# flybirdxx/ComfyUI-SDMatte

Measured on AMD Instinct MI355X. Metric: alpha mattes/sec at 1024x1024, higher is better.
Workload: dtype f16x3

## Files before the change

comfyui-sdmatte_amd/csrc/k_gemm.h:

```cpp
#pragma once
#include "sdm_common.h"

#ifndef P3_X8_TRUNC_GAIN
#define P3_X8_TRUNC_GAIN 1.097f
#endif

SDM_DEV_INLINE int p3_xl_pos(int c) { const int j = c >> 3; return ((j & 1) << 4) | ((j >> 1) << 3) | (c & 7); }
SDM_HD_INLINE size_t p3_rows_pad(size_t rows) { return (rows + 31) & ~(size_t)31; }
SDM_DEV_INLINE size_t p3_hi_off(size_t row, int C, int c) {
  return ((((row >> 4) * (size_t)(C >> 5)) + (size_t)(c >> 5)) << 10) + (size_t)((((c & 31) >> 3) << 8) + ((int)(row & 15) << 4));
}
SDM_DEV_INLINE size_t p3_xl_off(size_t row, int C, int c) {
  const int pos = p3_xl_pos(c & 31);
  return ((((row >> 5) * (size_t)(C >> 5)) + (size_t)(c >> 5)) << 10) + (size_t)(((pos >> 4) << 9) + ((int)(row & 31) << 4) + (pos & 15));
}

SDM_DEV_INLINE float p3_gelu(float g) {
  const float z = fabsf(g) * 0.70710678118654752f;
  const float t = sdm_rcp(1.0f + 0.3275911f * z);
  const float poly = t * (0.254829592f + t * (-0.284496736f + t * (1.421413741f + t * (-1.453152027f + t * 1.061405429f))));
  const float er = 1.0f - poly * sdm_exp2(-z * z * SDM_LOG2E);
  return 0.5f * g * (1.0f + copysignf(er, g));
}

// ... 1 lines not shown
  const half_t* a_hi; const unsigned char* a_xl;
  long M; int K;
  int rows_per_img;
  const unsigned char* w; int N;
  const float* bias;
  void* out; int ldo;
  int n_valid;
  size_t out_lo_off;
  int lo_cols;
  const float* res; int ldr;
  float* stats;
  int sa, sb;
  int tiles_m, tiles_n, xcd_chunk, tiles_per_img;
  int ablate;
  int up_H, up_W;
};

SDM_DEV_INLINE void p3_pack_block(const float (&v)[16], u32x4 (&hi)[2], u32x4& xl) {
  unsigned int H[4][2], X[4];
#pragma unroll
  for (int g = 0; g < 4; ++g) {
    float y[4], l[4];
    half_t hh[4];
#pragma unroll
    for (int e = 0; e < 4; ++e) {
      y[e] = SDM_MED3(v[4 * g + e], -57344.0f, 57344.0f);
      hh[e] = (half_t)y[e];
      l[e] = (y[e] - (float)hh[e]) * 2048.0f;
    }
    f16x2 p0, p1;
// ... 372 lines not shown
          const u32x4 hv = {H[2 * q][0], H[2 * q][1], H[2 * q + 1][0], H[2 * q + 1][1]};
          const u32x4 pv = {P[2 * q][0], P[2 * q][1], P[2 * q + 1][0], P[2 * q + 1][1]};
          sdm_buffer_store16(hv, rs_hi, ok ? (ro + (unsigned int)ch) * 2u : SDM_BUF_INVALID, 0);
          SDM_PIN_STORE_DATA(hv);
          sdm_buffer_store16(pv, rs_pr, (ok && ch < p.lo_cols) ? (ro + (unsigned int)ch) * 2u : SDM_BUF_INVALID, 0);
          SDM_PIN_STORE_DATA(pv);
        }
      }
    }
  }
  }
  v_cur = next_tile(v_cur + (int)gridDim.x, mt_c, nt_c);
  }
}

SDM_DEV_INLINE float up_phase_weight(const half_t* __restrict__ k_hi, const half_t* __restrict__ k_lo, int Cout_pad, int phase, int tap, int c, int co) {
  const int py = phase >> 1, px = phase & 1, a = tap >> 1, b = tap & 1;
  float s = 0.0f;
  for (int ky = 0; ky < 3; ++ky) {
    if (((py + ky + 1) >> 1) - 1 != py - 1 + a) continue;
    for (int kx = 0; kx < 3; ++kx) {
      if (((px + kx + 1) >> 1) - 1 != px - 1 + b) continue;
      const size_t si = (((size_t)(c / 16) * 9 + ky * 3 + kx) * Cout_pad + co) * 16 + (c % 16);
      s += (float)k_hi[si] + (float)k_lo[si];
    }
  }
  return s;
}
__global__ void up_phase_absmax_kernel(const half_t* __restrict__ k_hi, const half_t* __restrict__ k_lo, int Cin_pad, int Cout_pad, unsigned int* __restrict__ out) {
  const size_t n = (size_t)16 * Cin_pad * Cout_pad;
// ... 201 lines not shown
```

comfyui-sdmatte_amd/csrc/sdm_engine.cpp:

```cpp
#include "sdm_common.h"
#include "k_conv.h"
#include "k_gemm.h"
#include "k_norm.h"
#include "k_attn.h"
#include "k_misc.h"
#include "k_trimap.h"
#include "k_cclabel.h"
#include "k_foreground.h"
#include "k_guided.h"
#include "k_roi.h"
#include "k_canvas.h"
#include "k_boxes.h"
#include "k_distance.h"
#include "../../include/sdmatte.h"

#include <algorithm>
#include <cmath>
#include <cstdio>
#include <cstdlib>
#include <cstring>
#include <atomic>
#include <map>
#include <mutex>
#include <shared_mutex>
// ... 48 lines not shown
}
#endif
static inline size_t rupz(size_t a, size_t b) { return ((a + b - 1) / b) * b; }

struct OptEntry { const char* name; int value; int def; const char* what; };
static OptEntry g_opts[] = {
  {"conv_f8", 1, 1, "residual terms of the wide split-precision 3x3 convs on fp8 MFMAs (read when a model is built)"},
  {"gemm_f8", 1, 1, "the same for Linear / 1x1 layers with K >= gemm_f8_min_k (read when a model is built)"},
  {"gemm_f8_min_k", 1024, 1024, "smallest K of a GEMM that takes the 8-wave fp8-residual kernel"},
  {"gemm_p3", 1, 1, "transformer-block Linear layers on the plane-fed GEMM (k_gemm.h): pre-split operand planes from LayerNorm / GroupNorm / attention / GEGLU, LDS-DMA only (the W3 weight copies are built when a model is built)"},
  {"gemm_p3_tile", 0, 0, "row tile of the plane-fed GEMM: 0 by shape, 256 / 128 / 64 forced"},
  {"gemm_p3_attn", 1, 1, "d=64 attention cores write the operand planes of to_out themselves (0: fp32 result + one conversion pass)"},
  {"gemm_p3_persist", 1, 1, "plane-fed GEMM: persistent blocks that prefetch the next tile's first chunk underneath the epilogue (0: one block per tile, n > 1: a grid of n blocks - tests)"},
  {"gemm_p3_ablate", 0, 0, "bench only: 1 no MFMAs, 2 no DMAs behind the prologue, 4 no epilogue (sdm_bench_gemm_p3)"},
  {"conv_up_phase", 1, 1, "up-sampling 3x3 convs (Upsample2D) as four 2x2-tap phase convs on the plane-fed GEMM (k_gemm.h, UP): 0 off (the 3x3 kernels on the up-sampled image), 1 the launches with at least two 256-row tiles per CU (up_phase_wins: measured), 2 every eligible launch (tests).  0 / non-0 is read when a model is built: the phase matrices are a derived weight layout"},
  {"conv_epi", 4, 4, "F8 kernels' epilogue: 4 register-direct stores + residual as accumulator init, 3 residual init only, 0 LDS-staged"},
  {"conv_xtile", 1, 1, "F8 3x3: cross-tile prefetch by the producer waves"},
  {"conv_f8_tpb", 0, 0, "F8: tiles per block (0 = by queue depth)"},
  {"conv_dma", 1, 1, "3x3 stride-1 256x128 tile: weights by LDS-DMA"},
  {"conv_dma_all", 0, 0, "keep a stage-ordered weight copy for every wide 3x3 layer, not only the split-precision ones (read when a model is built)"},
  {"conv_pc", -1, -1, "producer / consumer form of the split-precision DMA kernel: -1 by channel count, 0 off, 1 on"},
  {"conv_pc_min_cin", 256, 256, "conv_pc = -1: smallest Cin that takes the producer / consumer form"},
  {"conv_db", 0, 0, "512x128 double-buffered tile where the queue is deep"},
  {"trimap_skip", 1, 1, "VAE encoder, trimap images: output tiles inside a constant region of the trimap are not multiplied (k_misc.h cmask_*; exact). 0 = every tile"},
  {"conv_band_rows", 0, 0, "tile rows per XCD band of the convs that leave constant tiles out (0 = by image height)"},
  {"trimap_skip_min_rows", 512, 512, "smallest output height at which constant tiles are left out (measured at 1024^2: the 1024- and 512-row levels gain 3.7 + 1.6 ms, the 256-row level loses 0.7: too few of its 32 x 128-pixel tiles lie inside one region)"},
  {"conv_splitk", -1, -1, "split-K of the register-staged conv / GEMM kernels: -1 by shape (few tiles, long K), 0 off, n >= 2 forced where the shape allows"},
  {"force_cfg0", 0, 0, "always the 256x128 tile for 3x3 stride 1 (tests: fused GroupNorm at tiny sizes)"},
  {"no_gn_fuse", 0, 0, "never fuse the GroupNorm apply into the consuming conv"},
  {"split_lds_pad", 0, 0, "extra dynamic LDS of the register-staged split kernels (forces one block per CU)"},
// ... 237 lines not shown

template <int MT, int EPI, int UP = 0>
static void launch_gemm_p3_t(GemmP3Params p, void* stream) {
  constexpr int BM = 64 * MT, NS = 2, SMEM = NS * (BM * 96 + 128 * 128);
  const long rows = p.rows_per_img ? (long)p.rows_per_img : p.M;
  p.tiles_per_img = (int)((rows + BM - 1) / BM);
  p.tiles_m = p.tiles_per_img * (p.rows_per_img ? (int)(p.M / p.rows_per_img) : 1);
  p.tiles_n = sdm_cdiv(p.N, 128) * (UP ? 4 : 1);
  unsigned grid;
  if (p.tiles_m >= 8) { p.xcd_chunk = (p.tiles_m + 7) / 8; grid = (unsigned)(8L * p.xcd_chunk * p.tiles_n); }
  else { p.xcd_chunk = 0; grid = (unsigned)(p.tiles_m * p.tiles_n); }
  if (const int pp = opt("gemm_p3_persist")) {
    const unsigned slots = pp > 1 ? (unsigned)pp : ((unsigned)(device_cus() * ((SMEM <= 80 * 1024) ? 2 : 1)) & ~7u);
    if (slots >= 1 && grid > slots) grid = slots;
  }
  auto k = gemm_p3_kernel<MT, 2, EPI, NS, UP>;
  SDM_SET_SMEM(k, SMEM);
#ifndef SDM_EMU
  if (opt("gemm_p3_ablate") & 256) {
    int nb = -1;
    (void)hipOccupancyMaxActiveBlocksPerMultiprocessor(&nb, k, 256, (size_t)SMEM);
    fprintf(stderr, "[gemm_p3] tile %d stages %d epi %d: %d bytes of LDS, %d blocks per CU, grid %u\n", BM, NS, EPI, SMEM, nb, grid);
  }
#endif
  SDM_LAUNCH(k, dim3(grid, 1, 1), dim3(256), (size_t)SMEM, stream, p);
}
template <int EPI>
static void launch_gemm_p3_e(const GemmP3Params& p, int bm, void* stream) {
  if (bm == 256) launch_gemm_p3_t<4, EPI>(p, stream);
  else if (bm == 128) launch_gemm_p3_t<2, EPI>(p, stream);
// ... 7 lines not shown
  const int cus = device_cus();
  for (int bm : {256, 128}) if (imgs * ((rows + bm - 1) / bm) * tn >= cus) return bm;
  return 64;
}
static void launch_gemm_p3(const GemmP3Params& p, int epi, void* stream) {
  const int bm = gemm_p3_pick_bm(p.M, p.N, p.rows_per_img);
  switch (epi) {
    case 0: launch_gemm_p3_e<0>(p, bm, stream); break;
    case 1: launch_gemm_p3_e<1>(p, bm, stream); break;
    case 2: launch_gemm_p3_e<2>(p, bm, stream); break;
    case 3: launch_gemm_p3_e<3>(p, bm, stream); break;
    default: launch_gemm_p3_e<4>(p, bm, stream); break;
  }
}

static void launch_gemm_p3_up(const GemmP3Params& p, int epi, int bm, void* stream) {
  if (epi == 4) {
    if (bm == 256) launch_gemm_p3_t<4, 4, 1>(p, stream); else if (bm == 128) launch_gemm_p3_t<2, 4, 1>(p, stream); else launch_gemm_p3_t<1, 4, 1>(p, stream);
  } else {
    if (bm == 256) launch_gemm_p3_t<4, 0, 1>(p, stream); else if (bm == 128) launch_gemm_p3_t<2, 0, 1>(p, stream); else launch_gemm_p3_t<1, 0, 1>(p, stream);
  }
}

static int launch_conv(int ntaps, int stride, int cfg, const ConvParams& p, void* stream) {
  if (ntaps == 9 && stride == 1) {
    switch (cfg) {
      case 0:
        if (p.w_dma) { launch_conv_dma(p, stream); return 0; }
        launch_conv_t<9, 1, 8, 32, 128, 16, 2, 2, 0, 1>(p, stream); return 0;
      case 1: launch_conv_t<9, 1, 4, 32, 64, 32, 4, 1>(p, stream); return 0;
      case 2: launch_conv_t<9, 1, 8, 8, 64, 16, 2, 1>(p, stream); return 0;
// ... 92 lines not shown
  return L;
}

static bool layer_takes_dma3x3(const ConvL& L) { return L.ntaps == 9 && L.Cout_pad >= 128 && !L.geglu; }
static bool layer_takes_gemm_f8(const ConvL& L) {
  return L.ntaps == 1 && L.split && L.Cout_pad >= 128 && L.Cin_pad % 32 == 0 && conv_f8_enabled() && gemm_f8_enabled();
}
static bool layer_takes_w3(const ConvL& L) { return L.ntaps == 1 && L.split && L.Cin_pad % 32 == 0 && L.Cin_pad >= 32; }
static bool layer_takes_up_phase(const ConvL& L) {
  return L.ntaps == 9 && L.split && !L.geglu && L.Cin_pad % 32 == 0 && L.Cin_pad >= 32 && conv_f8_enabled() && opt("conv_up_phase") != 0;
}
static bool up_phase_wins(int N, int H, int W, int Cout_pad) {
  if (opt("conv_up_phase") >= 2) return true;
  const long tiles = (long)N * sdm_cdiv((H + 2) * (W + 2), 256) * 4 * sdm_cdiv(Cout_pad, 128);
  return tiles >= 2L * device_cus();
}
static void layer_choose_layouts(ConvL& L, bool want_dma3x3, bool want_gemm_f8, bool want_w3, bool want_up_phase = false) {
  if (want_up_phase && layer_takes_up_phase(L)) L.wup_bytes = (size_t)16 * L.Cin_pad * L.Cout_pad * 4;
  if (want_dma3x3 && layer_takes_dma3x3(L)) {
    L.wdma_bytes = L.w_bytes() * (L.split ? 2 : 1);
    L.f8 = (L.split && L.Cin_pad % 32 == 0 && conv_f8_enabled()) ? 1 : 0;
  }
  if (want_gemm_f8 && layer_takes_gemm_f8(L)) { L.wdma_bytes = L.w_bytes() * 2; L.f8 = 1; }
  if (want_w3 && layer_takes_w3(L)) L.w3_bytes = L.w_bytes() * 2;
}
struct NormL {
  int C = 0;
  size_t g_off = 0, b_off = 0;
  float* g = nullptr;
  float* b = nullptr;
// ... 529 lines not shown
  return p3_rows_pad(rows) * (size_t)L.Cin_pad * 2 < SDM_BUF_INVALID && tile_out < SDM_BUF_INVALID && rows < ((size_t)1 << 31);
}
static int op_conv_up_phase(sdm_ctx* e, const ConvL& L, const ConvArgs& a) {
  const T& in = *a.in0;
  T* out = a.out;
  T xp = talloc(e, in.N, in.H + 2, in.W + 2, in.C, kFmtP3);
  GemmP3Params p;
  memset(&p, 0, sizeof(p));
  p.M = xp.rows(); p.K = L.Cin_pad; p.rows_per_img = (in.H + 2) * (in.W + 2);
  p.up_H = in.H; p.up_W = in.W;
  p.a_hi = (const half_t*)xp.p; p.a_xl = (const unsigned char*)xp.p + p3_rows_pad((size_t)p.M) * p.K * 2;
  p.w = L.wup; p.N = L.Cout_pad; p.bias = L.b;
  p.out = out->p; p.ldo = out->C; p.n_valid = a.cout_valid >= 0 ? a.cout_valid : std::min(L.Cout_pad, out->C);
  p.sa = 127 - 11; p.sb = 127 - L.up_exp;
  const int bm = gemm_p3_pick_bm(p.M, p.N, p.rows_per_img, 4);
  const int epi = out->want_stats ? 4 : 0;
  if (epi == 4) {
    out->srows = sdm_cdiv(p.rows_per_img, bm) * 8;
    T sb = talloc(e, 1, 1, 1, (int)((size_t)in.N * out->srows * out->C * 2), 1);
    out->soff = sb.off; out->sbytes = sb.bytes; out->stats = (float*)sb.p;
    p.stats = out->stats;
  }
  if (e->dry) { tfree(e, xp); return 0; }
  char d[256];
  d[0] = 0;
  if (e->prof_on) snprintf(d, sizeof(d), "%s N=%d H=%d W=%d C=%d bordered grid", L.name.c_str(), in.N, in.H, in.W, in.C);
  prof_begin(e, "to_p3", 0, (double)in.rows() * in.C * 4 + (double)xp.rows() * in.C * 3, d);
  const long units = ((xp.rows() + 31) / 32) * (in.C / 32);
  SDM_LAUNCH(to_p3_pad_kernel, dim3((unsigned)std::min<long>((units + 3) / 4, 1 << 20)), dim3(256), 0, e->stream, (const float*)in.p, (unsigned char*)xp.p, xp.rows(), in.C,
             in.H, in.W);
  prof_end(e);
  const double flops = 2.0 * (double)out->rows() * L.O * L.I * 4;
  const double bytes = (double)xp.rows() * p.K * 3 + (double)out->rows() * p.n_valid * 4 + (double)16 * p.K * p.N * 4;
  if (e->prof_on) {
    snprintf(d, sizeof(d), "%s N=%d Hout=%d Wout=%d Cin=%d Cout=%d up=1 phases epi=%d bm=%d", L.name.c_str(), in.N, out->H, out->W, L.Cin_pad, L.O, epi, bm);
    prof_begin(e, "conv_up_phase", flops, bytes, d);
  } else {
    prof_begin(e, "conv", flops, bytes);
  }
  count_kernel("conv_up_phase");
  launch_gemm_p3_up(p, epi, bm, e->stream);
#ifndef SDM_EMU
  { const hipError_t le = hipGetLastError(); if (le != hipSuccess) SDM_FAIL(e, SDM_ERR_HIP, "conv %s: launch failed: %s", L.name.c_str(), hipGetErrorString(le)); }
#endif
  prof_end(e);
  tfree(e, xp);
  return 0;
}

static int op_conv(sdm_ctx* e, const ConvL& L, const ConvArgs& a) {
  if (conv_up_phase_ok(L, a)) return op_conv_up_phase(e, L, a);
  ConvParams p;
  memset(&p, 0, sizeof(p));
  conv_shape_params(p, L, *a.in0, a.in1, *a.out, a.stride);
  p.in0 = a.in0->p;
  if (a.in1) p.in1 = a.in1->p;
// ... 2367 lines not shown
```

comfyui-sdmatte_amd/csrc/sdm_hooks.h:

```cpp
#pragma once

struct DevBuf {
  void* p = nullptr;
  DevBuf() = default;
  DevBuf(DevBuf&& o) noexcept : p(o.p) { o.p = nullptr; }
  ~DevBuf() { if (p) dev_free(p); }
  int alloc(size_t n) { return dev_malloc(&p, n); }
  int alloc0(size_t n, void* stream) { const int rc = alloc(n); return rc ? rc : dev_memset(p, 0, n, stream); }
};

struct RestoreInt { int& s; int v; ~RestoreInt() { s = v; } };

struct TempLayer {
  enum { kDma = 1, kW3 = 2, kUp = 4 };
  sdm_ctx* e;
  ConvL L;
  DevBuf w, w_lo, b, w_dma, w3, wup;
  explicit TempLayer(sdm_ctx* c) : e(c) {}
  ~TempLayer() { dev_sync(e->stream); }
  int init(const char* name, int ntaps, int I, int O, int geglu, int split, int layouts, const float* wsrc, const float* bias) {
    L = make_layer(name, ntaps, I, O, geglu, split);
    layer_choose_layouts(L, layouts & kDma, layouts & kDma, layouts & kW3, layouts & kUp);
    SDM_CHECK_DEV(e, w.alloc0(L.w_bytes(), e->stream));
    SDM_CHECK_DEV(e, b.alloc0(L.b_bytes(), e->stream));
// ... 209 lines not shown
  GemmP3Params p;
  memset(&p, 0, sizeof(p));
  p.M = M; p.K = K; p.a_hi = (const half_t*)xp.p; p.a_xl = (const unsigned char*)xp.p + p3_rows_pad((size_t)M) * K * 2;
  p.w = tl.L.w3; p.N = O; p.bias = tl.L.b; p.out = out.p; p.ldo = Cst; p.n_valid = Cst;
  p.out_lo_off = epi == 2 ? (size_t)M * Cst : p3_rows_pad((size_t)M) * Cst * 2; p.lo_cols = (O / 3) * 2;
  if (resf) { p.res = (const float*)resb.p; p.ldr = Cst; }
  if (epi == 4) { p.stats = (float*)st.p; p.rows_per_img = (int)M; }
  p.sa = 127 - 11; p.sb = 127 - tl.L.f8_exp; p.ablate = opt("gemm_p3_ablate");
  const float ms = time_launches(e, iters, [&]() { launch_gemm_p3(p, epi, e->stream); });
  const hipError_t le = hipGetLastError();
  if (le != hipSuccess) { e->err = hipGetErrorString(le); return -3.f; }
  return ms;
#endif
}

float sdm_bench_conv(sdm_ctx* e, int N, int H, int W, int Cin, int Cout, int ntaps, int stride, int in_f32, int tile_cfg, int ablate, int iters) {
  const int split = (in_f32 >> 1) & 1, gnf = (in_f32 >> 2) & 1, pcf = (in_f32 >> 3) & 1, f8f = (in_f32 >> 4) & 1;
  const int of32 = (in_f32 >> 5) & 1, resf = (in_f32 >> 6) & 1, statf = (in_f32 >> 7) & 1;
  in_f32 = (in_f32 & 1) | split;
  if (e) dev_use(e->device);
  if (!e) return -1.f;
#ifdef SDM_EMU
  return -1.f;
#else
  ConvL L;
  L.name = "bench"; L.ntaps = ntaps; L.I = Cin; L.O = Cout; L.Cin_pad = rup(Cin, 16); L.Cout_pad = rup(Cout, 32);
  DevBuf wp, bp, in, out, wl, gnt, resb, statb, wdm, wsb;
  const int Ho = stride == 2 ? H / 2 : H, Wo = stride == 2 ? W / 2 : W;
  const size_t wbytes = (size_t)L.Cin_pad * ntaps * L.Cout_pad * 2, inb = (size_t)N * H * W * L.Cin_pad * (in_f32 ? 4 : 2),
               outb = (size_t)N * Ho * Wo * L.Cout_pad * (of32 ? 4 : 2);
// ... 372 lines not shown
```

comfyui-sdmatte_amd/engine.py:

```python
import ctypes as C
import os

import numpy as np
import torch

from .config import SDMatteConfig

_HERE = os.path.dirname(os.path.abspath(__file__))
LIB_PATH = os.path.join(_HERE, "csrc", "libsdmatte_hip.so")

SDM_PTR_HOST, SDM_PTR_DEVICE = 0, 1
SDM_F32, SDM_F16, SDM_BF16 = 0, 1, 2
_DT = {torch.float32: SDM_F32, torch.float16: SDM_F16, torch.bfloat16: SDM_BF16}


class SdmConfig(C.Structure):
    _fields_ = [
        ("vae_channels", C.c_int32 * 4), ("vae_layers_per_block", C.c_int32),
        ("unet_channels", C.c_int32 * 4), ("unet_heads", C.c_int32 * 4), ("unet_layers_per_block", C.c_int32),
        ("cross_attention_dim", C.c_int32), ("unet_in_channels", C.c_int32), ("unet_out_channels", C.c_int32),
        ("bbox_embeddings_input_dim", C.c_int32), ("groups", C.c_int32),
        ("vae_eps", C.c_float), ("unet_res_eps", C.c_float), ("unet_tf_gn_eps", C.c_float), ("unet_ln_eps", C.c_float),
        ("vae_scaling_factor", C.c_float), ("attn_mask_value", C.c_float),
        ("stream_f32", C.c_int32), ("point_embeddings_input_dim", C.c_int32), ("precise_mask", C.c_int32), ("reserved", C.c_int32 * 5),
# ... 36 lines not shown
    c.unet_tf_gn_eps, c.unet_ln_eps = cfg.unet_tf_gn_eps, cfg.unet_ln_eps
    c.vae_scaling_factor, c.attn_mask_value = cfg.vae_scaling_factor, cfg.attn_mask_value
    c.stream_f32 = 1 if stream_f32 else 0
    c.point_embeddings_input_dim = cfg.point_embeddings_input_dim
    c.precise_mask = precise_mask_of(precision)
    return c


EXPORTS = [
    "sdm_default_config", "sdm_create", "sdm_destroy", "sdm_last_error", "sdm_load_tensor", "sdm_finalize_weights",
    "sdm_weight_stats", "sdm_missing_key", "sdm_weight_blob_bytes", "sdm_export_weight_blob", "sdm_import_weight_blob",
    "sdm_host_blob_bytes", "sdm_export_host_blob", "sdm_import_host_blob", "sdm_forward", "sdm_forward_ex", "sdm_forward_rect", "sdm_apply_matte", "sdm_apply_matte_node",
    "sdm_make_trimap", "sdm_clean_mask", "sdm_apply_matte_mask", "sdm_subject_roi", "sdm_apply_matte_roi", "sdm_subject_boxes", "sdm_apply_matte_boxes", "sdm_estimate_foreground", "sdm_refine_alpha_guided", "sdm_compose_canvas",
    "sdm_distance_field", "sdm_offset_mask", "sdm_outline",
    "sdm_synchronize", "sdm_release_memory", "sdm_resident_bytes", "sdm_weight_bytes", "sdm_last_forward_ms", "sdm_profile_enable", "sdm_profile_count", "sdm_profile_get", "sdm_profile_dump",
    "sdm_op_conv", "sdm_op_conv_ex", "sdm_op_conv_up_stats", "sdm_op_gemm_p3", "sdm_debug_run_layer", "sdm_debug_set_input_cmask", "sdm_debug_temb_row", "sdm_conv_num_cfgs", "sdm_bench_conv", "sdm_bench_attn", "sdm_bench_gemm_p3", "sdm_op_groupnorm", "sdm_op_layernorm", "sdm_op_attention", "sdm_op_attention_ex", "sdm_op_attention_split", "sdm_op_attention_split_ex", "sdm_debug_attn_plan", "sdm_op_resize_aa",
    "sdm_op_mask_bias", "sdm_op_cross_patch_planes", "sdm_op_cross_patch_planes_ex", "sdm_op_attention_shared", "sdm_debug_cross_attention", "sdm_op_cross_core",
    "sdm_set_option", "sdm_get_option", "sdm_reset_options", "sdm_option_name", "sdm_option_help", "sdm_kernel_counts", "sdm_kernel_counts_reset",
]


class Bindings:

    def __init__(self, cdll):
        self.dll = cdll
        vp, i32, i64, f32 = C.c_void_p, C.c_int, C.c_int64, C.c_float
        sig = {
            "sdm_default_config": (None, [C.POINTER(SdmConfig)]),
            "sdm_create": (i32, [C.POINTER(vp), i32, C.POINTER(SdmConfig)]),
            "sdm_destroy": (None, [vp]),
            "sdm_last_error": (C.c_char_p, [vp]),
# ... 36 lines not shown
            "sdm_profile_get": (i32, [vp, i32, C.POINTER(C.c_char_p), C.POINTER(f32), C.POINTER(i64), C.POINTER(C.c_double),
                                      C.POINTER(C.c_double)]),
            "sdm_op_conv": (i32, [vp, vp, vp, i32, i32, i32, i32, i32, i32, i32, i32, i32, i32, vp, vp, i32, vp, i32, vp, i32, i32,
                                  f32, i32]),
            "sdm_op_conv_ex": (i32, [vp, vp, vp, i32, i32, i32, i32, i32, i32, i32, i32, i32, i32, vp, vp, i32, vp, i32, vp, i32, i32,
                                     f32, i32, i32, vp, vp, f32, i32, i32]),
            "sdm_op_gemm_p3": (i32, [vp, vp, i32, i32, i32, i32, vp, vp, i32, i32, vp, vp, vp, f32, i32, vp, vp, C.POINTER(i32)]),
            "sdm_op_conv_up_stats": (i32, [vp, vp, i32, i32, i32, i32, vp, vp, i32, vp, vp, C.POINTER(i32)]),
            "sdm_debug_run_layer": (i32, [vp, C.c_char_p, vp, i32, i32, i32, vp, i32]),
            "sdm_debug_set_input_cmask": (i32, [vp, vp]),
            "sdm_debug_temb_row": (i32, [vp, i32, i32, vp, vp, i32]),
            "sdm_conv_num_cfgs": (i32, [i32, i32]),
            "sdm_bench_conv": (f32, [vp] + [i32] * 11),
            "sdm_bench_attn": (f32, [vp] + [i32] * 7),
            "sdm_bench_gemm_p3": (f32, [vp, C.c_long, i32, i32, i32, i32]),
            "sdm_op_groupnorm": (i32, [vp, vp, vp, i32, i32, i32, i32, i32, i32, vp, vp, f32, i32, vp]),
            "sdm_op_layernorm": (i32, [vp, vp, i32, C.c_long, i32, vp, vp, f32, vp]),
            "sdm_op_attention": (i32, [vp, vp, i32, vp, i32, vp, i32, vp, i32, i32, i32, i32, i32, vp, i32]),
            "sdm_op_attention_ex": (i32, [vp, vp, i32, vp, i32, vp, i32, i32, i32, i32, i32, i32, i32, vp, i32]),
            "sdm_op_attention_split": (i32, [vp, vp, vp, vp, vp, i32, i32, i32, i32, vp]),
            "sdm_op_attention_split_ex": (i32, [vp, vp, vp, vp, vp, vp, i32, i32, i32, i32, i32, vp, vp]),
            "sdm_debug_attn_plan": (i32, [i32] * 10 + [C.c_char_p, i32, C.POINTER(i32)]),
            "sdm_op_resize_aa": (i32, [vp, vp, i32, i32, i32, vp, i32, i32]),
            "sdm_op_mask_bias": (i32, [vp, vp, i32, i32, i32, vp]),
            "sdm_op_cross_patch_planes": (i32, [vp, vp, i32, i32, i32, vp, vp, vp]),
            "sdm_op_cross_patch_planes_ex": (i32, [vp, vp, i32, i32, i32, vp, vp, vp, i32]),
            "sdm_op_cross_core": (i32, [vp, vp, vp, i32, i32, i32, i32, i32, vp]),
            "sdm_op_attention_shared": (i32, [vp, vp, vp, vp, i32, i32, i32, i32, i32, vp]),
            "sdm_debug_cross_attention": (i32, [vp, C.c_char_p, vp, i32, i32, i32, vp, i32, i32, vp]),
            "sdm_set_option": (i32, [C.c_char_p, i32]),
# ... 760 lines not shown
        return out

    def debug_temb_row(self, index, is_trans, coords, cout):
        out = np.zeros(cout, np.float32)
        co = None if coords is None else np.ascontiguousarray(np.asarray(coords, np.float32).reshape(4))
        self._check(self.lib.sdm_debug_temb_row(self.h, index, int(is_trans), co.ctypes.data_as(C.c_void_p) if co is not None else None,
                                                out.ctypes.data_as(C.c_void_p), cout), "sdm_debug_temb_row")
        return torch.from_numpy(out)

    def bench_conv(self, N, H, W, Cin, Cout, ntaps=9, stride=1, in_f32=0, tile_cfg=-1, ablate=0, iters=10):
        return float(self.lib.sdm_bench_conv(self.h, N, H, W, Cin, Cout, ntaps, stride, in_f32, tile_cfg, ablate, iters))

    def bench_gemm_p3(self, M, K, O, epi=0, res=False, iters=10):
        return float(self.lib.sdm_bench_gemm_p3(self.h, M, K, O, epi | (256 if res else 0), iters))

    def bench_attn(self, B, heads, Lq, Lk, qt=1, ablate=0, iters=10):
        return float(self.lib.sdm_bench_attn(self.h, B, heads, Lq, Lk, qt, ablate, iters))

    def op_groupnorm(self, x0, gamma, beta, eps, silu, groups=32, x1=None):
        N, H, W_, C0 = x0.shape
        C1 = x1.shape[-1] if x1 is not None else 0
        out = torch.empty(N, H, W_, C0 + C1, dtype=torch.float16, device=x0.device)
        self._check(self.lib.sdm_op_groupnorm(self.h, _ptr(x0), _ptr(x1), C0, C1, int(x0.dtype == torch.float32), N, H * W_, groups,
                                              _ptr(gamma), _ptr(beta), float(eps), int(silu), _ptr(out)), "sdm_op_groupnorm")
        return out

    def op_layernorm(self, x, gamma, beta, eps):
        rows, Cc = x.numel() // x.shape[-1], x.shape[-1]
        out = torch.empty(x.shape, dtype=torch.float16, device=x.device)
        self._check(self.lib.sdm_op_layernorm(self.h, _ptr(x), int(x.dtype == torch.float32), rows, Cc, _ptr(gamma), _ptr(beta),
# ... 81 lines not shown
```

include/sdmatte.h:

```cpp
#ifndef SDMATTE_H_
#define SDMATTE_H_

#include <stddef.h>
#include <stdint.h>

#ifdef __cplusplus
extern "C" {
#endif

typedef struct sdm_ctx sdm_ctx;

enum sdm_status {
  SDM_OK = 0,
  SDM_ERR_INVALID = -1,
  SDM_ERR_HIP = -2,
  SDM_ERR_STATE = -3,
  SDM_ERR_NOMEM = -4,
  SDM_ERR_NODEVICE = -5,
  SDM_ERR_ARENA = -6
};

enum sdm_ptr_kind { SDM_PTR_HOST = 0, SDM_PTR_DEVICE = 1 };
enum sdm_dtype { SDM_F32 = 0, SDM_F16 = 1, SDM_BF16 = 2 };

// ... 146 lines not shown
int sdm_profile_enable(sdm_ctx* ctx, int on);
int sdm_profile_count(sdm_ctx* ctx);
const char* sdm_profile_dump(sdm_ctx* ctx);
int sdm_profile_get(sdm_ctx* ctx, int i, const char** name, float* ms, int64_t* launches, double* flops, double* bytes);


int sdm_op_conv(sdm_ctx* ctx, const void* in0, const void* in1, int C0, int C1, int in_f32, int N, int Hin, int Win, int up,
                int stride, int pad_mode, int ntaps, const float* w, const float* bias, int O, void* out, int out_f32,
                const void* res, int res_f32, int geglu, float out_scale, int tile_cfg);
int sdm_conv_num_cfgs(int ntaps, int stride);
int sdm_op_conv_ex(sdm_ctx* ctx, const void* in0, const void* in1, int C0, int C1, int in_f32, int N, int Hin, int Win, int up,
                   int stride, int pad_mode, int ntaps, const float* w, const float* bias, int O, void* out, int out_f32,
                   const void* res, int res_f32, int geglu, float out_scale, int tile_cfg, int split, const float* gn_gamma,
                   const float* gn_beta, float gn_eps, int gn_groups, int gn_silu);
float sdm_bench_gemm_p3(sdm_ctx* ctx, long M, int K, int O, int epi_flags, int iters);
int sdm_op_gemm_p3(sdm_ctx* ctx, const float* x, int N, int H, int W, int K, const float* w, const float* bias, int O, int mode, const float* res,
                   const float* ln_gamma, const float* ln_beta, float ln_eps, int lo_cols, void* out, float* stats, int* srows);
int sdm_op_conv_up_stats(sdm_ctx* ctx, const float* x, int N, int H, int W, int C, const float* w, const float* bias, int O, float* out, float* stats,
                         int* srows);
int sdm_debug_set_input_cmask(sdm_ctx* ctx, const unsigned char* mask);
int sdm_debug_run_layer(sdm_ctx* ctx, const char* layer_name, const float* x_nhwc, int N, int H, int W, float* out_nhwc, int Cout);
int sdm_debug_temb_row(sdm_ctx* ctx, int temb_index, int is_trans, const float* coords4, float* out_host, int cout);
float sdm_bench_attn(sdm_ctx* ctx, int B, int heads, int Lq, int Lk, int qt, int ablate, int iters);
float sdm_bench_conv(sdm_ctx* ctx, int N, int H, int W, int Cin, int Cout, int ntaps, int stride, int in_f32, int tile_cfg, int ablate, int iters);
int sdm_op_groupnorm(sdm_ctx* ctx, const void* in0, const void* in1, int C0, int C1, int in_f32, int N, int HW, int groups,
                     const float* gamma, const float* beta, float eps, int silu, void* out_f16);
int sdm_op_layernorm(sdm_ctx* ctx, const void* x, int in_f32, long rows, int C, const float* gamma, const float* beta,
                     float eps, void* out_f16);
int sdm_op_attention(sdm_ctx* ctx, const void* q, int ldq, const void* k, int ldk, const void* v, int ldv, const float* bias,
                     int B, int heads, int Lq, int Lk, int D, void* out, int ldo);
// ... 20 lines not shown
```

Measured before the change: 21.98.

## Add halo-tile kernel for up-sampling phase convs sharing LDS activations across taps

Adds gemm_p3_up_halo_kernel. It loads one (TH+1)x33 activation halo tile into LDS per channel chunk and reuses it for all four 2x2 taps of a phase conv, instead of reading a separate row tile per tap. This is meant to cut global and LDS-DMA traffic for the activation operand of the Upsample2D convs. It uses a ring of weight slots, tuned vmcnt waits and a statistics layout per spatial tile. The cost is a larger LDS footprint, possibly lower occupancy, and partial tiles at image edges. It is enabled by default for launches with at least two tiles per CU, and also adds a benchmark entry point and a grid-cap test option.

```diff
diff --git a/comfyui-sdmatte_amd/csrc/k_gemm.h b/comfyui-sdmatte_amd/csrc/k_gemm.h
--- a/comfyui-sdmatte_amd/csrc/k_gemm.h
+++ b/comfyui-sdmatte_amd/csrc/k_gemm.h
@@ -39,6 +39,7 @@
   int tiles_m, tiles_n, xcd_chunk, tiles_per_img;
   int ablate;
   int up_H, up_W;
+  int up_tw;
 };
 
 SDM_DEV_INLINE void p3_pack_block(const float (&v)[16], u32x4 (&hi)[2], u32x4& xl) {
@@ -441,6 +442,292 @@
   }
 }
 
+template <int V> struct p3_ic { static constexpr int v = V; };
+template <int N> SDM_DEV_INLINE void p3_wait_vmcnt() {
+#ifndef SDM_EMU
+  asm volatile("s_waitcnt vmcnt(%0)" :: "n"(N) : "memory");
+#endif
+}
+template <int TH, int NW> struct P3HaloCfg {
+  static constexpr int MT = TH / 2, BN = 128;
+  static constexpr int RH = (TH + 1) * 33, ND = (RH + 63) / 64, RPAD = ND * 64;
+  static constexpr int A_HI = 4 * RPAD * 16, A_BUF = 6 * RPAD * 16, W_SLOT = BN * 128, OFF_W = 2 * A_BUF, SMEM = OFF_W + NW * W_SLOT;
+};
+template <int TH, int NW, int EPI>
+__global__ void __launch_bounds__(256, (P3HaloCfg<TH, NW>::SMEM <= 80 * 1024) ? 2 : 1) gemm_p3_up_halo_kernel(GemmP3Params p) {
+  using CF = P3HaloCfg<TH, NW>;
+  constexpr int MT = CF::MT, NT = 2, BN = CF::BN, ND = CF::ND, RPAD = CF::RPAD, RH = CF::RH;
+  constexpr int A_HI = CF::A_HI, A_BUF = CF::A_BUF, W_SLOT = CF::W_SLOT, OFF_W = CF::OFF_W, B_HI = BN * 64;
+  constexpr int AW = (6 * ND + 3) / 4, NXW = AW - ND, NWI = 2 * (BN / 16 / 4);
+  constexpr int AP0 = (AW + 2) / 3, AP1 = (AW + 1) / 3, AP2 = AW / 3;
+  constexpr int AL0 = (NW == 2) ? 0 : NWI, AL1 = (NW == 2) ? AP0 : NWI + AP0, AL2 = (NW == 2) ? AP1 : AP0 + NWI + AP1, AL3 = (NW == 2) ? AP2 : AP1 + NWI + AP2;
+  static_assert(TH % 2 == 0 && (NW == 2 || NW == 3) && AP0 + AP1 + AP2 == AW && NXW >= 1 && NXW * 4 <= 4 * ND && AL2 <= 63 && AL3 <= 63, "halo tile / ring");
+  static_assert(EPI == 0 || EPI == 4, "up-sampling phase convs store fp32 rows");
+  SDM_DYN_SMEM(smem);
+  const int tx = (int)threadIdx.x, lane = tx & 63, wave = SDM_UNIFORM_I(tx >> 6);
+  const int wm = wave >> 1, wn = wave & 1, h = lane >> 5, l31 = lane & 31;
+  const int nchunk = p.K >> 5, nch = nchunk * 4;
+  const unsigned int K = (unsigned int)p.K, N = (unsigned int)p.N;
+  const int up_wp = p.up_W + 2, up_tn = p.tiles_n >> 2;
+  const long rows_pad = (long)p3_rows_pad((size_t)p.M);
+  const int vgrid = (p.xcd_chunk > 0) ? 8 * p.xcd_chunk * p.tiles_n : p.tiles_m * p.tiles_n;
+  auto next_tile = [&](int v, int& mt, int& nt) -> int {
+    for (; v < vgrid; v += (int)gridDim.x) {
+      if (p.xcd_chunk > 0) {
+        const int j = v >> 3, ml = j / p.tiles_n;
+        nt = j - ml * p.tiles_n;
+        mt = (v & 7) * p.xcd_chunk + ml;
+        if (mt < p.tiles_m) return v;
+      } else {
+        mt = v / p.tiles_n;
+        nt = v - mt * p.tiles_n;
+        return v;
+      }
+    }
+    return -1;
+  };
+  auto tile_org = [&](int mt, int& img, int& mti, int& y0, int& x0) {
+    img = mt / p.tiles_per_img; mti = mt - img * p.tiles_per_img;
+    const int tyi = mti / p.up_tw;
+    y0 = tyi * TH; x0 = (mti - tyi * p.up_tw) * 32;
+  };
+  const sdm_rsrc rs_ahi = sdm_make_rsrc(p.a_hi, (unsigned int)rows_pad * K * 2u);
+  const sdm_rsrc rs_axl = sdm_make_rsrc(p.a_xl, (unsigned int)rows_pad * K);
+  const unsigned int vo_w = (unsigned int)lane * 16u;
+
+  unsigned int hi_vo[ND], xl_vo[NXW];
+  int xl_dst[NXW];
+#pragma unroll
+  for (int k = 0; k < NXW; ++k) {
+    int q = k * 4 + wave;
+    if (q >= 2 * ND) q -= 2 * ND;
+    xl_dst[k] = A_HI + (q & 1) * RPAD * 16 + (q >> 1) * 1024;
+  }
+  auto a_setup = [&](int mt, int ph) {
+    int img, mti, y0, x0;
+    tile_org(mt, img, mti, y0, x0);
+    const int yb0 = y0 + (ph >> 1), xb0 = x0 + (ph & 1);
+    auto src_row = [&](int R, bool& ok) -> size_t {
+      const int r = R / 33, s = R - r * 33, yb = yb0 + r, xb = xb0 + s;
+      ok = R < RH && yb <= p.up_H + 1 && xb <= p.up_W + 1;
+      return (size_t)img * p.rows_per_img + (size_t)yb * up_wp + xb;
+    };
+#pragma unroll
+    for (int k = 0; k < ND; ++k) {
+      bool ok;
+      const size_t row = src_row(k * 64 + lane, ok);
+      hi_vo[k] = ok ? (unsigned int)p3_hi_off(row, (int)K, wave * 8) : SDM_BUF_INVALID;
+    }
+#pragma unroll
+    for (int k = 0; k < NXW; ++k) {
+      int q = k * 4 + wave;
+      if (q >= 2 * ND) q -= 2 * ND;
+      bool ok;
+      const size_t row = src_row((q >> 1) * 64 + lane, ok);
+      xl_vo[k] = ok ? (unsigned int)p3_xl_off(row, (int)K, (q & 1) * 8) : SDM_BUF_INVALID;
+    }
+  };
+  int mt_c, nt_c, v_cur = next_tile((int)blockIdx.x, mt_c, nt_c);
+  if (v_cur < 0) return;
+  auto nt_phase = [&](int nt) -> int { return nt / up_tn; };
+  auto nt_col0 = [&](int nt) -> int { return (nt % up_tn) * BN; };
+  int v_a = v_cur, cc_a = 0, par_a = 0;
+  a_setup(mt_c, nt_phase(nt_c));
+  auto issue_a = [&](auto part) {
+    constexpr int T = decltype(part)::v;
+    constexpr int A0 = (T == 0) ? 0 : (T == 1) ? AP0 : AP0 + AP1, AN = (T == 0) ? AP0 : (T == 1) ? AP1 : AP2;
+    if (v_a < 0) return;
+    unsigned char* ab = smem + par_a * A_BUF;
+    const unsigned int add = (unsigned int)cc_a << 10;
+#pragma unroll
+    for (int a = A0; a < A0 + AN; ++a) {
+      if (a < ND) {
+        sdm_glds16_buf(rs_ahi, hi_vo[a] == SDM_BUF_INVALID ? SDM_BUF_INVALID : hi_vo[a] + add, 0u, ab + wave * (RPAD * 16) + a * 1024);
+      } else {
+        sdm_glds16_buf(rs_axl, xl_vo[a - ND] == SDM_BUF_INVALID ? SDM_BUF_INVALID : xl_vo[a - ND] + add, 0u, ab + xl_dst[a - ND]);
+      }
+    }
+    if (T == 2) {
+      par_a ^= 1;
+      if (++cc_a == nchunk) {
+        int mt, nt;
+        cc_a = 0;
+        v_a = next_tile(v_a + (int)gridDim.x, mt, nt);
+        if (v_a >= 0) a_setup(mt, nt_phase(nt));
+      }
+    }
+  };
+  int v_w = v_cur, s_w = 0, slot_w = 0, n0_w = nt_col0(nt_c), ph_w = nt_phase(nt_c);
+  auto issue_w = [&]() {
+    if (v_w < 0) return;
+    unsigned char* st = smem + OFF_W + slot_w * W_SLOT;
+    const sdm_rsrc rs_wc = sdm_make_rsrc(p.w + (size_t)ph_w * ((size_t)nch * N * 128u), (unsigned int)nch * N * 128u);
+    const unsigned int wb = (unsigned int)s_w * N * 128u + (unsigned int)n0_w * 64u;
+#pragma unroll
+    for (int i0 = 0; i0 < BN / 16; i0 += 4) {
+      const int i = i0 + wave;
+      sdm_glds16_buf(rs_wc, vo_w, wb + (unsigned int)i * 1024u, st + i * 1024);
+    }
+#pragma unroll
+    for (int i0 = 0; i0 < BN / 16; i0 += 4) {
+      const int i = i0 + wave;
+      sdm_glds16_buf(rs_wc, vo_w, wb + N * 64u + (unsigned int)i * 1024u, st + B_HI + i * 1024);
+    }
+    slot_w = (slot_w + 1 == NW) ? 0 : slot_w + 1;
+    if (++s_w == nch) {
+      int mt, nt;
+      s_w = 0;
+      v_w = next_tile(v_w + (int)gridDim.x, mt, nt);
+      if (v_w >= 0) { n0_w = nt_col0(nt); ph_w = nt_phase(nt); }
+    }
+  };
+  issue_a(p3_ic<0>()); issue_a(p3_ic<1>()); issue_a(p3_ic<2>());
+#pragma unroll
+  for (int s = 0; s < NW - 1; ++s) issue_w();
+
+  f32x16 acc[MT][NT];
+  int wh_off[NT], w8_off[NT], ah_off[MT];
+#pragma unroll
+  for (int j = 0; j < NT; ++j) {
+    const int nb = wn * NT + j;
+    wh_off[j] = (((nb * 2 + (l31 >> 4)) * 4 + h) * 256) + (lane & 15) * 16;
+    w8_off[j] = B_HI + ((nb * 4 + h) * 512) + l31 * 16;
+  }
+#pragma unroll
+  for (int i = 0; i < MT; ++i) ah_off[i] = (h * RPAD + (wm * MT + i) * 33 + l31) * 16;
+  const int sa8 = p.sa, sb8 = p.sb;
+  const bool ab_mm = (p.ablate & 1) != 0, ab_dma = (p.ablate & 2) != 0;
+  int par_c = 0, slot_c = 0;
+  bool first = true;
+  while (v_cur >= 0) {
+  int img, mti, y0, x0;
+  tile_org(mt_c, img, mti, y0, x0);
+  const int n0 = nt_col0(nt_c), phase = nt_phase(nt_c);
+#pragma unroll
+  for (int i = 0; i < MT; ++i)
+#pragma unroll
+    for (int j = 0; j < NT; ++j)
+#pragma unroll
+      for (int r = 0; r < 16; ++r) acc[i][j][r] = 0.0f;
+  for (int cc = 0; cc < nchunk; ++cc) {
+    const unsigned char* ab = smem + par_c * A_BUF;
+    par_c ^= 1;
+    auto step = [&](auto tapc) {
+      constexpr int T = decltype(tapc)::v;
+      constexpr int TAP_OFF = ((T >> 1) * 33 + (T & 1)) * 16;
+      if (first || v_a < 0) SDM_WAIT_VMCNT0();
+      else p3_wait_vmcnt<(T == 0) ? AL0 : (T == 1) ? AL1 : (T == 2) ? AL2 : AL3>();
+      SDM_RAW_BARRIER();
+      if (!ab_dma) {
+        issue_w();
+        if (T < 3) issue_a(p3_ic<(T < 3) ? T : 0>());
+      }
+      first = false;
+      const unsigned char* st = smem + OFF_W + slot_c * W_SLOT;
+      slot_c = (slot_c + 1 == NW) ? 0 : slot_c + 1;
+      if (ab_mm && (cc > 0 || T > 0)) return;
+      f16x8 wh[2][NT];
+      i32x8 w8[NT];
+#pragma unroll
+      for (int j = 0; j < NT; ++j) {
+        wh[0][j] = *(const f16x8*)(st + wh_off[j]);
+        wh[1][j] = *(const f16x8*)(st + wh_off[j] + 512);
+        const i32x4 q0 = *(const i32x4*)(st + w8_off[j]), q1 = *(const i32x4*)(st + w8_off[j] + 1024);
+        w8[j] = i32x8{q0[0], q0[1], q0[2], q0[3], q1[0], q1[1], q1[2], q1[3]};
+      }
+      constexpr int RP = (MT % 2 == 0) ? 2 : MT;
+#pragma unroll
+      for (int i0 = 0; i0 < MT; i0 += RP) {
+        f16x8 a0[RP], a1[RP];
+        i32x8 a8[RP];
+#pragma unroll
+        for (int r = 0; r < RP; ++r) {
+          const unsigned char* ap = ab + ah_off[i0 + r] + TAP_OFF;
+          a0[r] = *(const f16x8*)ap; a1[r] = *(const f16x8*)(ap + 2 * RPAD * 16);
+          const i32x4 xl = *(const i32x4*)(ap + A_HI);
+          const u32x4 u0 = __builtin_bit_cast(u32x4, a0[r]), u1 = __builtin_bit_cast(u32x4, a1[r]);
+          a8[r][0] = xl[0]; a8[r][1] = xl[1]; a8[r][2] = xl[2]; a8[r][3] = xl[3];
+          a8[r][4] = (int)sdm_perm_b32(u0[1], u0[0], 0x07050301u); a8[r][5] = (int)sdm_perm_b32(u0[3], u0[2], 0x07050301u);
+          a8[r][6] = (int)sdm_perm_b32(u1[1], u1[0], 0x07050301u); a8[r][7] = (int)sdm_perm_b32(u1[3], u1[2], 0x07050301u);
+        }
+#pragma unroll
+        for (int r = 0; r < RP; ++r)
+#pragma unroll
+          for (int j = 0; j < NT; ++j) acc[i0 + r][j] = SDM_MFMA_32x32x16_F16(wh[0][j], a0[r], acc[i0 + r][j]);
+#pragma unroll
+        for (int r = 0; r < RP; ++r)
+#pragma unroll
+          for (int j = 0; j < NT; ++j) acc[i0 + r][j] = SDM_MFMA_32x32x16_F16(wh[1][j], a1[r], acc[i0 + r][j]);
+#pragma unroll
+        for (int r = 0; r < RP; ++r)
+#pragma unroll
+          for (int j = 0; j < NT; ++j) acc[i0 + r][j] = SDM_MFMA_32x32x64_F8A_BF8B(w8[j], a8[r], acc[i0 + r][j], sb8, sa8);
+      }
+    };
+    step(p3_ic<0>()); step(p3_ic<1>()); step(p3_ic<2>()); step(p3_ic<3>());
+  }
+
+  if (p.ablate & 4) { if (acc[0][0][0] == 123.456f) ((float*)p.out)[0] = 1.0f; }
+  else {
+  const float* bias = p.bias;
+  f32x4 bq[NT][4];
+#pragma unroll
+  for (int j = 0; j < NT; ++j)
+#pragma unroll
+    for (int g = 0; g < 4; ++g) {
+      const int ch = n0 + (wn * NT + j) * 32 + 8 * g + 4 * h;
+      bq[j][g] = (bias && ch < p.N) ? *(const f32x4*)(bias + ch) : f32x4{0.0f, 0.0f, 0.0f, 0.0f};
+    }
+  const int py = phase >> 1, px = phase & 1;
+  const int th_live = (p.up_H - y0) < TH ? (p.up_H - y0) : TH;
+  const size_t orow = (size_t)2 * p.up_W * p.ldo;
+  const float* obase = (const float*)p.out + ((size_t)img * 2 * p.up_H + 2 * (size_t)y0) * orow;
+  const sdm_rsrc rs_out = sdm_make_rsrc(obase, (unsigned int)((size_t)2 * th_live * orow * 4));
+  unsigned int ro[MT];
+#pragma unroll
+  for (int i = 0; i < MT; ++i) {
+    const int ty = wm * MT + i, x = x0 + l31;
+    ro[i] = (ty < th_live && x < p.up_W) ? (((unsigned int)(2 * ty + py) * 2u * (unsigned int)p.up_W + 2u * (unsigned int)x + (unsigned int)px) * (unsigned int)p.ldo) * 4u : SDM_BUF_INVALID;
+  }
+  constexpr bool do_stats = (EPI == 4);
+  const size_t prow = (size_t)img * (p.tiles_per_img * 8) + ((size_t)mti * 4 + phase) * 2 + wm;
+#pragma unroll
+  for (int jg = 0; jg < NT * 4; ++jg) {
+    const int j = jg >> 2, g = jg & 3;
+    const int ch = n0 + (wn * NT + j) * 32 + 8 * g + 4 * h;
+    float t1[4] = {0.0f, 0.0f, 0.0f, 0.0f}, t2[4] = {0.0f, 0.0f, 0.0f, 0.0f};
+#pragma unroll
+    for (int i = 0; i < MT; ++i) {
+      f32x4 v;
+#pragma unroll
+      for (int e = 0; e < 4; ++e) v[e] = acc[i][j][4 * g + e] + bq[j][g][e];
+      const bool live = ro[i] != SDM_BUF_INVALID;
+      sdm_buffer_store16(__builtin_bit_cast(u32x4, v), rs_out, (ch < p.n_valid && live) ? ro[i] + (unsigned int)ch * 4u : SDM_BUF_INVALID, 0);
+      if (do_stats && live) {
+#pragma unroll
+        for (int e = 0; e < 4; ++e) { t1[e] += v[e]; t2[e] += v[e] * v[e]; }
+      }
+      SDM_PIN_STORE_DATA(v);
+    }
+    if (do_stats) {
+#pragma unroll
+      for (int e = 0; e < 4; ++e) {
+        t1[e] = sdm_sum_row16(t1[e]); t2[e] = sdm_sum_row16(t2[e]);
+        t1[e] += __shfl_xor(t1[e], 16); t2[e] += __shfl_xor(t2[e], 16);
+      }
+      if (l31 == 0 && ch < p.n_valid) {
+        float* dst = p.stats + (prow * p.ldo + ch) * 2;
+        *(f32x4*)dst = f32x4{t1[0], t2[0], t1[1], t2[1]};
+        *(f32x4*)(dst + 4) = f32x4{t1[2], t2[2], t1[3], t2[3]};
+      }
+    }
+  }
+  }
+  first = true;
+  v_cur = next_tile(v_cur + (int)gridDim.x, mt_c, nt_c);
+  }
+}
+
 SDM_DEV_INLINE float up_phase_weight(const half_t* __restrict__ k_hi, const half_t* __restrict__ k_lo, int Cout_pad, int phase, int tap, int c, int co) {
   const int py = phase >> 1, px = phase & 1, a = tap >> 1, b = tap & 1;
   float s = 0.0f;
diff --git a/comfyui-sdmatte_amd/csrc/sdm_engine.cpp b/comfyui-sdmatte_amd/csrc/sdm_engine.cpp
--- a/comfyui-sdmatte_amd/csrc/sdm_engine.cpp
+++ b/comfyui-sdmatte_amd/csrc/sdm_engine.cpp
@@ -86,6 +86,9 @@
   {"gemm_p3_persist", 1, 1, "plane-fed GEMM: persistent blocks that prefetch the next tile's first chunk underneath the epilogue (0: one block per tile, n > 1: a grid of n blocks - tests)"},
   {"gemm_p3_ablate", 0, 0, "bench only: 1 no MFMAs, 2 no DMAs behind the prologue, 4 no epilogue (sdm_bench_gemm_p3)"},
   {"conv_up_phase", 1, 1, "up-sampling 3x3 convs (Upsample2D) as four 2x2-tap phase convs on the plane-fed GEMM (k_gemm.h, UP): 0 off (the 3x3 kernels on the up-sampled image), 1 the launches with at least two 256-row tiles per CU (up_phase_wins: measured), 2 every eligible launch (tests).  0 / non-0 is read when a model is built: the phase matrices are a derived weight layout"},
+  {"conv_up_halo", 1, 1, "phase convs with one activation halo tile in LDS for the four taps of a channel chunk (k_gemm.h, gemm_p3_up_halo_kernel): 0 the flat form, 1 where it measured faster (up_halo_tile: the launches with at least two 256-row tiles per CU), 2 every phase launch (tests)"},
+  {"conv_up_halo_tile", 0, 0, "halo form: source rows of the M tile: 0 = 6, 8 (256 pixels, 3 weight slots, one block per CU) / 6 (192 pixels, 2 weight slots, two blocks per CU) forced"},
+  {"gemm_p3_max_blocks", 0, 0, "tests: at most this many blocks per phase-conv launch (0 = off), so that one block of a small launch walks several tiles"},
   {"conv_epi", 4, 4, "F8 kernels' epilogue: 4 register-direct stores + residual as accumulator init, 3 residual init only, 0 LDS-staged"},
   {"conv_xtile", 1, 1, "F8 3x3: cross-tile prefetch by the producer waves"},
   {"conv_f8_tpb", 0, 0, "F8: tiles per block (0 = by queue depth)"},
@@ -353,6 +356,7 @@
     const unsigned slots = pp > 1 ? (unsigned)pp : ((unsigned)(device_cus() * ((SMEM <= 80 * 1024) ? 2 : 1)) & ~7u);
     if (slots >= 1 && grid > slots) grid = slots;
   }
+  if (UP) { const int cap = opt("gemm_p3_max_blocks"); if (cap > 0 && grid > (unsigned)cap) grid = (unsigned)cap; }
   auto k = gemm_p3_kernel<MT, 2, EPI, NS, UP>;
   SDM_SET_SMEM(k, SMEM);
 #ifndef SDM_EMU
@@ -390,7 +394,28 @@
   }
 }
 
-static void launch_gemm_p3_up(const GemmP3Params& p, int epi, int bm, void* stream) {
+template <int TH, int NW, int EPI>
+static void launch_gemm_p3_up_halo_t(GemmP3Params p, void* stream) {
+  constexpr int SMEM = P3HaloCfg<TH, NW>::SMEM;
+  p.up_tw = sdm_cdiv(p.up_W, 32);
+  p.tiles_per_img = sdm_cdiv(p.up_H, TH) * p.up_tw;
+  p.tiles_m = p.tiles_per_img * (int)(p.M / p.rows_per_img);
+  p.tiles_n = sdm_cdiv(p.N, 128) * 4;
+  unsigned grid;
+  if (p.tiles_m >= 8) { p.xcd_chunk = (p.tiles_m + 7) / 8; grid = (unsigned)(8L * p.xcd_chunk * p.tiles_n); }
+  else { p.xcd_chunk = 0; grid = (unsigned)(p.tiles_m * p.tiles_n); }
+  if (const int pp = opt("gemm_p3_persist")) {
+    const unsigned slots = pp > 1 ? (unsigned)pp : ((unsigned)(device_cus() * ((SMEM <= 80 * 1024) ? 2 : 1)) & ~7u);
+    if (slots >= 1 && grid > slots) grid = slots;
+  }
+  { const int cap = opt("gemm_p3_max_blocks"); if (cap > 0 && grid > (unsigned)cap) grid = (unsigned)cap; }
+  auto k = gemm_p3_up_halo_kernel<TH, NW, EPI>;
+  SDM_SET_SMEM(k, SMEM);
+  SDM_LAUNCH(k, dim3(grid, 1, 1), dim3(256), (size_t)SMEM, stream, p);
+}
+static void launch_gemm_p3_up(const GemmP3Params& p, int epi, int bm, void* stream, int halo_th = 0) {
+  if (halo_th == 8) { if (epi == 4) launch_gemm_p3_up_halo_t<8, 3, 4>(p, stream); else launch_gemm_p3_up_halo_t<8, 3, 0>(p, stream); return; }
+  if (halo_th == 6) { if (epi == 4) launch_gemm_p3_up_halo_t<6, 2, 4>(p, stream); else launch_gemm_p3_up_halo_t<6, 2, 0>(p, stream); return; }
   if (epi == 4) {
     if (bm == 256) launch_gemm_p3_t<4, 4, 1>(p, stream); else if (bm == 128) launch_gemm_p3_t<2, 4, 1>(p, stream); else launch_gemm_p3_t<1, 4, 1>(p, stream);
   } else {
@@ -513,6 +538,16 @@
   if (opt("conv_up_phase") >= 2) return true;
   const long tiles = (long)N * sdm_cdiv((H + 2) * (W + 2), 256) * 4 * sdm_cdiv(Cout_pad, 128);
   return tiles >= 2L * device_cus();
+}
+static int up_halo_tile(int N, int H, int W, int Cout_pad, int out_C) {
+  const int o = opt("conv_up_halo");
+  if (o == 0) return 0;
+  const int forced = opt("conv_up_halo_tile");
+  const int th = (forced == 8 || forced == 6) ? forced : 6;
+  if ((size_t)2 * th * 2 * W * out_C * 4 >= SDM_BUF_INVALID) return 0;
+  if (o >= 2) return th;
+  const long tiles = (long)N * sdm_cdiv((H + 2) * (W + 2), 256) * 4 * sdm_cdiv(Cout_pad, 128);
+  return tiles >= 2L * device_cus() ? th : 0;
 }
 static void layer_choose_layouts(ConvL& L, bool want_dma3x3, bool want_gemm_f8, bool want_w3, bool want_up_phase = false) {
   if (want_up_phase && layer_takes_up_phase(L)) L.wup_bytes = (size_t)16 * L.Cin_pad * L.Cout_pad * 4;
@@ -1072,9 +1107,10 @@
   p.out = out->p; p.ldo = out->C; p.n_valid = a.cout_valid >= 0 ? a.cout_valid : std::min(L.Cout_pad, out->C);
   p.sa = 127 - 11; p.sb = 127 - L.up_exp;
   const int bm = gemm_p3_pick_bm(p.M, p.N, p.rows_per_img, 4);
+  const int halo = up_halo_tile(in.N, in.H, in.W, L.Cout_pad, out->C);
   const int epi = out->want_stats ? 4 : 0;
   if (epi == 4) {
-    out->srows = sdm_cdiv(p.rows_per_img, bm) * 8;
+    out->srows = (halo ? sdm_cdiv(in.H, halo) * sdm_cdiv(in.W, 32) : sdm_cdiv(p.rows_per_img, bm)) * 8;
     T sb = talloc(e, 1, 1, 1, (int)((size_t)in.N * out->srows * out->C * 2), 1);
     out->soff = sb.off; out->sbytes = sb.bytes; out->stats = (float*)sb.p;
     p.stats = out->stats;
@@ -1091,13 +1127,14 @@
   const double flops = 2.0 * (double)out->rows() * L.O * L.I * 4;
   const double bytes = (double)xp.rows() * p.K * 3 + (double)out->rows() * p.n_valid * 4 + (double)16 * p.K * p.N * 4;
   if (e->prof_on) {
-    snprintf(d, sizeof(d), "%s N=%d Hout=%d Wout=%d Cin=%d Cout=%d up=1 phases epi=%d bm=%d", L.name.c_str(), in.N, out->H, out->W, L.Cin_pad, L.O, epi, bm);
+    snprintf(d, sizeof(d), "%s N=%d Hout=%d Wout=%d Cin=%d Cout=%d up=1 phases epi=%d bm=%d halo=%d", L.name.c_str(), in.N, out->H, out->W, L.Cin_pad, L.O, epi, bm, halo);
     prof_begin(e, "conv_up_phase", flops, bytes, d);
   } else {
     prof_begin(e, "conv", flops, bytes);
   }
   count_kernel("conv_up_phase");
-  launch_gemm_p3_up(p, epi, bm, e->stream);
+  if (halo) count_kernel("conv_up_halo");
+  launch_gemm_p3_up(p, epi, bm, e->stream, halo);
 #ifndef SDM_EMU
   { const hipError_t le = hipGetLastError(); if (le != hipSuccess) SDM_FAIL(e, SDM_ERR_HIP, "conv %s: launch failed: %s", L.name.c_str(), hipGetErrorString(le)); }
 #endif
diff --git a/comfyui-sdmatte_amd/csrc/sdm_hooks.h b/comfyui-sdmatte_amd/csrc/sdm_hooks.h
--- a/comfyui-sdmatte_amd/csrc/sdm_hooks.h
+++ b/comfyui-sdmatte_amd/csrc/sdm_hooks.h
@@ -247,6 +247,45 @@
 #endif
 }
 
+float sdm_bench_conv_up(sdm_ctx* e, int N, int H, int W, int C, int O, int epi, int iters) {
+  if (e) dev_use(e->device);
+  if (!e || C % 32 || O % 32 || (epi != 0 && epi != 4)) return -1.f;
+#ifdef SDM_EMU
+  (void)N; (void)H; (void)W; (void)iters;
+  return -1.f;
+#else
+  const size_t rows_in = (size_t)N * H * W, rows = (size_t)N * (H + 2) * (W + 2), rows_out = rows_in * 4;
+  DevBuf xf, xp, out, st;
+  if (xf.alloc(rows_in * C * 4) || xp.alloc(p3_rows_pad(rows) * C * 3) || out.alloc(rows_out * O * 4 + 256)) return -2.f;
+  if (epi == 4 && st.alloc((size_t)N * (8 * (((size_t)(H + 2) * (W + 2) + 63) / 64) + 8) * O * 8)) return -2.f;
+  SDM_LAUNCH(fill_random_f32_kernel, dim3(4096), dim3(256), 0, e->stream, (float*)xf.p, (long)(rows_in * C), 5u, 1.0f);
+  const long units = (long)((rows + 31) / 32) * (C / 32);
+  SDM_LAUNCH(to_p3_pad_kernel, dim3((unsigned)std::min<long>((units + 3) / 4, 1 << 20)), dim3(256), 0, e->stream, (const float*)xf.p, (unsigned char*)xp.p, (long)rows, C, H, W);
+  TempLayer tl(e);
+  {
+    DevBuf wf;
+    if (wf.alloc((size_t)9 * C * O * 4)) return -2.f;
+    SDM_LAUNCH(fill_random_f32_kernel, dim3(2048), dim3(256), 0, e->stream, (float*)wf.p, (long)9 * C * O, 17u, 0.05f);
+    if (tl.init("bench_up", 9, C, O, 0, 1, TempLayer::kUp, (const float*)wf.p, nullptr) != 0 || !tl.L.wup) return -2.f;
+  }
+  GemmP3Params p;
+  memset(&p, 0, sizeof(p));
+  p.M = (long)rows; p.K = tl.L.Cin_pad; p.rows_per_img = (H + 2) * (W + 2);
+  p.up_H = H; p.up_W = W;
+  p.a_hi = (const half_t*)xp.p; p.a_xl = (const unsigned char*)xp.p + p3_rows_pad(rows) * p.K * 2;
+  p.w = tl.L.wup; p.N = tl.L.Cout_pad; p.bias = tl.L.b;
+  p.out = out.p; p.ldo = O; p.n_valid = O;
+  p.sa = 127 - 11; p.sb = 127 - tl.L.up_exp; p.ablate = opt("gemm_p3_ablate");
+  if (epi == 4) p.stats = (float*)st.p;
+  const int bm = gemm_p3_pick_bm(p.M, p.N, p.rows_per_img, 4);
+  const int halo = up_halo_tile(N, H, W, tl.L.Cout_pad, O);
+  const float ms = time_launches(e, iters, [&]() { launch_gemm_p3_up(p, epi, bm, e->stream, halo); });
+  const hipError_t le = hipGetLastError();
+  if (le != hipSuccess) { e->err = hipGetErrorString(le); return -3.f; }
+  return ms;
+#endif
+}
+
 float sdm_bench_conv(sdm_ctx* e, int N, int H, int W, int Cin, int Cout, int ntaps, int stride, int in_f32, int tile_cfg, int ablate, int iters) {
   const int split = (in_f32 >> 1) & 1, gnf = (in_f32 >> 2) & 1, pcf = (in_f32 >> 3) & 1, f8f = (in_f32 >> 4) & 1;
   const int of32 = (in_f32 >> 5) & 1, resf = (in_f32 >> 6) & 1, statf = (in_f32 >> 7) & 1;
diff --git a/comfyui-sdmatte_amd/engine.py b/comfyui-sdmatte_amd/engine.py
--- a/comfyui-sdmatte_amd/engine.py
+++ b/comfyui-sdmatte_amd/engine.py
@@ -74,7 +74,7 @@
     "sdm_make_trimap", "sdm_clean_mask", "sdm_apply_matte_mask", "sdm_subject_roi", "sdm_apply_matte_roi", "sdm_subject_boxes", "sdm_apply_matte_boxes", "sdm_estimate_foreground", "sdm_refine_alpha_guided", "sdm_compose_canvas",
     "sdm_distance_field", "sdm_offset_mask", "sdm_outline",
     "sdm_synchronize", "sdm_release_memory", "sdm_resident_bytes", "sdm_weight_bytes", "sdm_last_forward_ms", "sdm_profile_enable", "sdm_profile_count", "sdm_profile_get", "sdm_profile_dump",
-    "sdm_op_conv", "sdm_op_conv_ex", "sdm_op_conv_up_stats", "sdm_op_gemm_p3", "sdm_debug_run_layer", "sdm_debug_set_input_cmask", "sdm_debug_temb_row", "sdm_conv_num_cfgs", "sdm_bench_conv", "sdm_bench_attn", "sdm_bench_gemm_p3", "sdm_op_groupnorm", "sdm_op_layernorm", "sdm_op_attention", "sdm_op_attention_ex", "sdm_op_attention_split", "sdm_op_attention_split_ex", "sdm_debug_attn_plan", "sdm_op_resize_aa",
+    "sdm_op_conv", "sdm_op_conv_ex", "sdm_op_conv_up_stats", "sdm_op_gemm_p3", "sdm_debug_run_layer", "sdm_debug_set_input_cmask", "sdm_debug_temb_row", "sdm_conv_num_cfgs", "sdm_bench_conv", "sdm_bench_attn", "sdm_bench_gemm_p3", "sdm_bench_conv_up", "sdm_op_groupnorm", "sdm_op_layernorm", "sdm_op_attention", "sdm_op_attention_ex", "sdm_op_attention_split", "sdm_op_attention_split_ex", "sdm_debug_attn_plan", "sdm_op_resize_aa",
     "sdm_op_mask_bias", "sdm_op_cross_patch_planes", "sdm_op_cross_patch_planes_ex", "sdm_op_attention_shared", "sdm_debug_cross_attention", "sdm_op_cross_core",
     "sdm_set_option", "sdm_get_option", "sdm_reset_options", "sdm_option_name", "sdm_option_help", "sdm_kernel_counts", "sdm_kernel_counts_reset",
 ]
@@ -141,6 +141,7 @@
             "sdm_bench_conv": (f32, [vp] + [i32] * 11),
             "sdm_bench_attn": (f32, [vp] + [i32] * 7),
             "sdm_bench_gemm_p3": (f32, [vp, C.c_long, i32, i32, i32, i32]),
+            "sdm_bench_conv_up": (f32, [vp, i32, i32, i32, i32, i32, i32, i32]),
             "sdm_op_groupnorm": (i32, [vp, vp, vp, i32, i32, i32, i32, i32, i32, vp, vp, f32, i32, vp]),
             "sdm_op_layernorm": (i32, [vp, vp, i32, C.c_long, i32, vp, vp, f32, vp]),
             "sdm_op_attention": (i32, [vp, vp, i32, vp, i32, vp, i32, vp, i32, i32, i32, i32, i32, vp, i32]),
@@ -931,6 +932,9 @@
     def bench_gemm_p3(self, M, K, O, epi=0, res=False, iters=10):
         return float(self.lib.sdm_bench_gemm_p3(self.h, M, K, O, epi | (256 if res else 0), iters))
 
+    def bench_conv_up(self, N, H, W, Cin, Cout, epi=4, iters=10):
+        return float(self.lib.sdm_bench_conv_up(self.h, N, H, W, Cin, Cout, epi, iters))
+
     def bench_attn(self, B, heads, Lq, Lk, qt=1, ablate=0, iters=10):
         return float(self.lib.sdm_bench_attn(self.h, B, heads, Lq, Lk, qt, ablate, iters))
 
diff --git a/include/sdmatte.h b/include/sdmatte.h
--- a/include/sdmatte.h
+++ b/include/sdmatte.h
@@ -184,6 +184,7 @@
                    const void* res, int res_f32, int geglu, float out_scale, int tile_cfg, int split, const float* gn_gamma,
                    const float* gn_beta, float gn_eps, int gn_groups, int gn_silu);
 float sdm_bench_gemm_p3(sdm_ctx* ctx, long M, int K, int O, int epi_flags, int iters);
+float sdm_bench_conv_up(sdm_ctx* ctx, int N, int H, int W, int C, int O, int epi, int iters);
 int sdm_op_gemm_p3(sdm_ctx* ctx, const float* x, int N, int H, int W, int K, const float* w, const float* bias, int O, int mode, const float* res,
                    const float* ln_gamma, const float* ln_beta, float ln_eps, int lo_cols, void* out, float* stats, int* srows);
 int sdm_op_conv_up_stats(sdm_ctx* ctx, const float* x, int N, int H, int W, int C, const float* w, const float* bias, int O, float* out, float* stats,
```

Result: no change. 22.08, median of 6 (+0.5%).
